# gevaertlab/sequoia-pub

Measured on AMD Instinct MI355X. Metric: slides/sec (1000-patch WSI, UNI-dim, 20k-gene head), higher is better.
Workload: dtype f16x3; 1 GPU; pipeline: 1000 x 224x224 uint8 patches/slide -> ResNet-50 embed -> k-Means(100) -> ViS(D=2048, depth 6, 16 heads, G=20820) forward (BASELINE config 3), patches uploaded from pinned host memory every step; embedder=ResNet-50 (src/resnet.py forward_extract), feature_dim=2048, patch_size=224, parallelism=slide-sharded x1

## Files before the change

### sequoia-pub_amd/csrc/gemm.h

```cpp
#pragma once
#include "sq_common.h"

#define SQ_ACT_NONE 0
#define SQ_ACT_GELU 1
#define SQ_ACT_RELU 2

struct GemmArgs {
    const void* A = nullptr;
    const void* B = nullptr;
    void* C = nullptr;
    bf16_t* C2 = nullptr;
    void* Cpre = nullptr;
    const float* bias = nullptr;
    const float* rowbias = nullptr;
    const void* res = nullptr;
    const void* gelu_grad_of = nullptr;
    const float* ln64_g = nullptr;
    const float* ln64_b = nullptr;
    float alpha = 1.0f;
    float* colsum_a = nullptr;
    int M = 0, N = 0, K = 0;
    int lda = 0, ldb = 0, ldc = 0, ldc2 = 0, ldpre = 0, ldres = 0, ldrb = 0, ldgg = 0;
    int rows_per_group = 1;
    int act = SQ_ACT_NONE;
    int out_dtype = SQ_F32, res_dtype = SQ_F32, pre_dtype = SQ_F32, gg_dtype = SQ_F32;
    int batch = 1;
    long long sA = 0, sB = 0, sC = 0, sC2 = 0, sPre = 0, sBias = 0, sRb = 0, sRes = 0, sGg = 0;
    int conv = 0, H = 0, W = 0, Cin = 0, OH = 0, OW = 0, KW = 1, stride = 1, pad = 0;
    size_t a_bytes = 0, b_bytes = 0;
    long long plA = 0, plB = 0, plRes = 0, plC = 0;
    int x3_f16 = 0;
    const float* colscale = nullptr;
    float* splitk_ws = nullptr;
    size_t splitk_ws_bytes = 0;
    int splitk = 1;
    int ngroup = 0;
    const void* gA[4] = {nullptr, nullptr, nullptr, nullptr};
    const void* gB[4] = {nullptr, nullptr, nullptr, nullptr};
    void* gC[4] = {nullptr, nullptr, nullptr, nullptr};
    float* gcs[4] = {nullptr, nullptr, nullptr, nullptr};
    int vec_epi = 0;
    int b_tiled = 0;
    const void* A2 = nullptr; long long plA2 = 0; size_t a2_bytes = 0; int lda2 = 0;
    const void* B2 = nullptr; size_t b2_bytes = 0; int ldb2 = 0; int K2 = 0;
    const float* bias2 = nullptr; const float* colscale2 = nullptr;
    int dH = 0, dW = 0, dOH = 0, dOW = 0, dstride = 1;
    int tile_group_m = 0;
    const void* comb_w = nullptr;
    const float* comb_rb = nullptr;
    int comb_ldrb = 0, comb_rpg = 1;
    int dbg = 0;
};

template <typename P>
static __device__ __forceinline__ P sq_group_pick(P const (&a)[4], int i) { return i == 0 ? a[0] : i == 1 ? a[1] : i == 2 ? a[2] : a[3]; }

int sq_launch_gemm(const GemmArgs& a, int dtype, hipStream_t stream);
bool sq_gemm_takes_p8_256(const GemmArgs& a);
int sq_launch_gemm_x3(const GemmArgs& a, hipStream_t stream);
int sq_launch_gemm_tn(const GemmArgs& a, int dtype, hipStream_t stream);
int sq_launch_splitk_reduce(const GemmArgs& a, hipStream_t stream);
```

### sequoia-pub_amd/csrc/gemm_x3.hip

```cpp
#include "gemm.h"
#include "x3_fmt.h"
#include "cdna_prims.h"

#include <cstdio>
#include <cstdlib>

extern int g_x3_small_max_k;
bool sq_conv_halo_x3_eligible(const GemmArgs& a);
int sq_launch_conv_halo_x3(const GemmArgs& a, hipStream_t stream);
extern int g_x3_halo;
extern int g_dbg;

namespace {

__device__ __forceinline__ u32x4 ld16(const bf16_t* p) { return *reinterpret_cast<const u32x4*>(p); }
__device__ __forceinline__ void st16(bf16_t* p, const u32x4& v) { *reinterpret_cast<u32x4*>(p) = v; }

constexpr int BK = 32, ROWB = 64;
constexpr int WTM = 2;

template <int BM_, int WTN> struct X3Cfg {
    static constexpr int BM = BM_;
    static constexpr int NT = BM_ * 2;
    static constexpr int BN = 64 * WTN;
    static constexpr int A_BYTES = BM * ROWB;
    static constexpr int B_BYTES = BN * ROWB;
    static constexpr int STAGE_BYTES = 2 * A_BYTES + 2 * B_BYTES;
    static constexpr int NSTAGE = BM_ == 256 ? 3 : 2;
    static constexpr int EPI_BYTES = BM * BN * 4;
    static constexpr int LDS_BYTES = NSTAGE * STAGE_BYTES > EPI_BYTES ? NSTAGE * STAGE_BYTES : EPI_BYTES;
    static constexpr int ROUND = NT / 4;
    static constexpr bool SPLIT_B = BN < ROUND;
    static constexpr int RB = SPLIT_B ? 1 : 2 * (BN / ROUND);
    static constexpr int LOADS = 4 + RB;
};

template <int BM_, int WTN, bool CONV, bool F16, bool PP, bool DUAL = false, bool UNI = false>
__global__ __launch_bounds__(BM_ * 2, BM_ == 256 ? 1 : 2) void gemm_x3_kernel(const GemmArgs p) {
    static_assert(!DUAL || (BM_ == 128 && !CONV && !PP), "the dual form lives in the 128-row two-stage shape");
    static_assert(!UNI || (F16 && !CONV && !DUAL), "the UNI epilogues are fp16-plane plain products");
    using Cfg = X3Cfg<BM_, WTN>;
    using Fmt = X3Fmt<F16>;
    constexpr int BM = Cfg::BM, NT = Cfg::NT, A_BYTES = Cfg::A_BYTES, ROUND = Cfg::ROUND;
    constexpr int BN = Cfg::BN, B_BYTES = Cfg::B_BYTES, STAGE_BYTES = Cfg::STAGE_BYTES, NSTAGE = Cfg::NSTAGE;
    static_assert(!PP || BM_ == 256, "the ping-pong schedule needs the 8-wave block");
    extern __shared__ __attribute__((aligned(16))) char smem[];

    const int tid = threadIdx.x, lane = tid & 63;
    const int wave = __builtin_amdgcn_readfirstlane(tid >> 6);
    const int wm = wave >> 1, wn = wave & 1;

    const int tiles_n = (p.N + BN - 1) / BN, tiles_m = (p.M + BM - 1) / BM;
    const int nwg = tiles_m * tiles_n;
    const int t = sq_xcd_tile(blockIdx.x, nwg);
    const int m0 = (t / tiles_n) * BM, n0 = (t % tiles_n) * BN;

    const bf16_t* Ah = reinterpret_cast<const bf16_t*>(p.A);
    const bf16_t* Bh = reinterpret_cast<const bf16_t*>(p.B);
    const auto rsAh = sq_rsrc(Ah, (int)p.a_bytes);
    const auto rsAl = sq_rsrc(Ah + p.plA, (int)p.a_bytes);
    const auto rsBh = sq_rsrc(Bh, (int)p.b_bytes);
    const auto rsBl = sq_rsrc(Bh + p.plB, (int)p.b_bytes);

    const int r0 = tid >> 2;
    const int gc = (tid & 3) ^ ((r0 >> 2) & 3);
    uint32_t a_off[2];
    int a_ih0[2], a_iw0[2];
    uint32_t a_pix[2];
    bool a_ok[2];
#pragma unroll
    for (int j = 0; j < 2; ++j) {
        const int m = m0 + r0 + ROUND * j;
        a_ok[j] = m < p.M;
        if constexpr (CONV) {
            const int ohw = p.OH * p.OW;
            const int img = m / ohw;
            const int rem = m - img * ohw;
            const int oh = rem / p.OW, ow = rem - oh * p.OW;
            a_ih0[j] = oh * p.stride - p.pad;
            a_iw0[j] = ow * p.stride - p.pad;
            a_pix[j] = (uint32_t)(img * p.H * p.W);
            a_off[j] = 0;
        } else {
            a_ih0[j] = a_iw0[j] = 0;
            a_pix[j] = 0;
            a_off[j] = a_ok[j] ? ((uint32_t)m * (uint32_t)p.lda + (uint32_t)(gc * 8)) * 2u : SQ_OOB;
        }
    }
    constexpr int RBP = Cfg::SPLIT_B ? 1 : BN / ROUND;
    uint32_t b_off[RBP];
    const bool b_lo_half = Cfg::SPLIT_B && r0 >= 64;
#pragma unroll
    for (int j = 0; j < RBP; ++j) {
        const int n = n0 + (Cfg::SPLIT_B ? (r0 & 63) : r0 + ROUND * j);
        b_off[j] = n >= p.N ? SQ_OOB : p.b_tiled ? ((uint32_t)n * 32u + (uint32_t)(gc * 8)) * 2u : ((uint32_t)n * (uint32_t)p.ldb + (uint32_t)(gc * 8)) * 2u;
    }
    auto issue_loads = [&](int kt, int buf) {
        const int k0 = kt * BK;
        const bool k_ok = k0 + gc * 8 < p.K;
        char* sa = smem + buf * STAGE_BYTES + wave * 1024;
        char* sb = sa + 2 * A_BYTES;
        if constexpr (CONV) {
            const int tap = k0 / p.Cin;
            const int cin0 = k0 - tap * p.Cin + gc * 8;
            const int kh = tap / p.KW, kw = tap - kh * p.KW;
#pragma unroll
// ... 282 lines not shown
            }
#pragma unroll
            for (int j = 0; j < WTN; ++j) {
                const int col = min(n0 + wn * (WTN * 32) + j * 32 + l31, p.N - 1);
                const float s3 = p.colscale ? p.alpha * p.colscale[col] : p.alpha, b3 = p.bias ? p.bias[col] : 0.f;
                const float sd = p.colscale2 ? p.colscale2[col] : 1.f, bd = p.bias2 ? p.bias2[col] : 0.f;
#pragma unroll
                for (int i = 0; i < WTM; ++i)
#pragma unroll
                    for (int r = 0; r < 16; r += 2) {
                        const float d0 = sd * accd[i][j][r] + bd, d1 = sd * accd[i][j][r + 1] + bd;
                        const uint32_t h = Fmt::pack2(d0, d1);
                        const uint32_t l = Fmt::rest2(d0, d1, h);
                        acc[i][j][r] = x3_relu((s3 * acc[i][j][r] + b3) + Fmt::sum_lo(h, l));
                        acc[i][j][r + 1] = x3_relu((s3 * acc[i][j][r + 1] + b3) + Fmt::sum_hi(h, l));
                    }
            }
        }
    }
    __syncthreads();

    float* stage = reinterpret_cast<float*>(smem);
#pragma unroll
    for (int i = 0; i < WTM; ++i)
#pragma unroll
        for (int j = 0; j < WTN; ++j)
#pragma unroll
            for (int r = 0; r < 16; ++r) {
                const int row = wm * (WTM * 32) + i * 32 + (r & 3) + 8 * (r >> 2) + 4 * lh;
                const int col = wn * (WTN * 32) + j * 32 + l31;
                stage[row * BN + col] = acc[i][j][r];
            }
    __syncthreads();
    if (!e_live) return;

    const bf16_t* resh = (!UNI && p.res) ? reinterpret_cast<const bf16_t*>(p.res) : nullptr;
    const float* res32 = (UNI && p.res) ? reinterpret_cast<const float*>(p.res) : nullptr;
    bf16_t* ch = p.out_dtype != SQ_F32 ? reinterpret_cast<bf16_t*>(p.C) : nullptr;
    float* c32 = p.out_dtype == SQ_F32 ? reinterpret_cast<float*>(p.C) : nullptr;
    constexpr int U = 4;
    u32x4 nh[U], nl[U];
    const bool res_nxt = res_pre && ITER == 2 * U && NPRE == U;
    if (res_nxt) {
#pragma unroll
        for (int u = 0; u < U; ++u) {
            const int m = min(m0 + e_rbase + (U + u) * RPI, p.M - 1);
            nh[u] = ld16(resh + (long long)m * p.ldres + e_n);
            nl[u] = ld16(resh + p.plRes + (long long)m * p.ldres + e_n);
        }
    }
#pragma unroll
    for (int c0 = 0; c0 < ITER; c0 += U) {
        u32x4 rh[U], rl[U];
#pragma unroll
        for (int u = 0; u < U; ++u) {
            rh[u] = u32x4{0, 0, 0, 0}; rl[u] = u32x4{0, 0, 0, 0};
            const int m = m0 + e_rbase + (c0 + u) * RPI;
            if constexpr (BM_ == 128) {
                if (res_pre && c0 + u < NPRE) { rh[u] = rpre_h[c0 + u]; rl[u] = rpre_l[c0 + u]; continue; }
                if (res_nxt && c0 == U) { rh[u] = nh[u]; rl[u] = nl[u]; continue; }
            }
            if (resh && m < p.M) {
                rh[u] = ld16(resh + (long long)m * p.ldres + e_n);
                rl[u] = ld16(resh + p.plRes + (long long)m * p.ldres + e_n);
            }
        }
#pragma unroll
        for (int u = 0; u < U; ++u) {
            const int row = e_rbase + (c0 + u) * RPI;
            const int m = m0 + row;
            if (m >= p.M) continue;
            const f32x4 a0 = *reinterpret_cast<const f32x4*>(stage + row * BN + e_c8 * 8);
            const f32x4 a1 = *reinterpret_cast<const f32x4*>(stage + row * BN + e_c8 * 8 + 4);
            float v[8] = {a0[0], a0[1], a0[2], a0[3], a1[0], a1[1], a1[2], a1[3]};
            if constexpr (!DUAL) {
#pragma unroll
            for (int e = 0; e < 8; ++e) v[e] = scale8[e] * v[e] + bias8[e];
            if (resh) {
                float idn[8];
                x3_join8<F16>(rh[u], rl[u], idn);
#pragma unroll
                for (int e = 0; e < 8; ++e) v[e] += idn[e];
            }
            if constexpr (UNI) {
                if (res32) {
                    const float* r = res32 + (long long)m * p.ldres + e_n;
                    const f32x4 r0 = *reinterpret_cast<const f32x4*>(r), r1 = *reinterpret_cast<const f32x4*>(r + 4);
#pragma unroll
                    for (int e = 0; e < 4; ++e) { v[e] += r0[e]; v[4 + e] += r1[e]; }
                }
                if (p.act == SQ_ACT_GELU) {
#pragma unroll
                    for (int e = 0; e < 8; ++e) v[e] = sq_gelu<false>(v[e]);
                }
            }
            if (p.act == SQ_ACT_RELU) {
#pragma unroll
                for (int e = 0; e < 8; ++e) v[e] = x3_relu(v[e]);
            }
            }
            if (p.dbg & 1) continue;
            if (c32) {
                float* d = c32 + (long long)m * p.ldc + e_n;
                *reinterpret_cast<f32x4*>(d) = f32x4{v[0], v[1], v[2], v[3]};
                *reinterpret_cast<f32x4*>(d + 4) = f32x4{v[4], v[5], v[6], v[7]};
            }
            if (ch) {
                u32x4 hi, lo;
                x3_split8<F16>(v, hi, lo);
                st16(ch + (long long)m * p.ldc + e_n, hi);
                st16(ch + p.plC + (long long)m * p.ldc + e_n, lo);
            }
        }
    }
}

template <int BM_, int WTN, bool F16, bool PP>
int launch_x3(const GemmArgs& a, hipStream_t stream) {
    using Cfg = X3Cfg<BM_, WTN>;
    static SqDevOnce attr;
    if (attr.needed()) {
        SQ_HIP_CHECK(hipFuncSetAttribute((const void*)gemm_x3_kernel<BM_, WTN, false, F16, PP>, hipFuncAttributeMaxDynamicSharedMemorySize, Cfg::LDS_BYTES));
        SQ_HIP_CHECK(hipFuncSetAttribute((const void*)gemm_x3_kernel<BM_, WTN, true, F16, PP>, hipFuncAttributeMaxDynamicSharedMemorySize, Cfg::LDS_BYTES));
        attr.done();
    }
    const int tiles = ((a.M + BM_ - 1) / BM_) * ((a.N + Cfg::BN - 1) / Cfg::BN);
    const dim3 grid(tiles), block(Cfg::NT);
    if (a.conv) hipLaunchKernelGGL((gemm_x3_kernel<BM_, WTN, true, F16, PP>), grid, block, Cfg::LDS_BYTES, stream, a);
    else hipLaunchKernelGGL((gemm_x3_kernel<BM_, WTN, false, F16, PP>), grid, block, Cfg::LDS_BYTES, stream, a);
    SQ_LAUNCH_CHECK();
    return SQ_OK;
}

template <bool F16>
int launch_x3_dual(const GemmArgs& a, hipStream_t stream) {
    using Cfg = X3Cfg<128, 2>;
    static SqDevOnce attr;
    if (attr.needed()) {
        SQ_HIP_CHECK(hipFuncSetAttribute((const void*)gemm_x3_kernel<128, 2, false, F16, false, true>, hipFuncAttributeMaxDynamicSharedMemorySize, Cfg::LDS_BYTES));
        attr.done();
    }
    const int tiles = ((a.M + 127) / 128) * (a.N / Cfg::BN);
    hipLaunchKernelGGL((gemm_x3_kernel<128, 2, false, F16, false, true>), dim3(tiles), dim3(Cfg::NT), Cfg::LDS_BYTES, stream, a);
    SQ_LAUNCH_CHECK();
    return SQ_OK;
}

template <int BM_, int WTN, bool PP>
int launch_x3_uni(const GemmArgs& a, hipStream_t stream) {
    using Cfg = X3Cfg<BM_, WTN>;
    static SqDevOnce attr;
    if (attr.needed()) {
        SQ_HIP_CHECK(hipFuncSetAttribute((const void*)gemm_x3_kernel<BM_, WTN, false, true, PP, false, true>, hipFuncAttributeMaxDynamicSharedMemorySize, Cfg::LDS_BYTES));
        attr.done();
    }
    const int tiles = ((a.M + BM_ - 1) / BM_) * ((a.N + Cfg::BN - 1) / Cfg::BN);
    hipLaunchKernelGGL((gemm_x3_kernel<BM_, WTN, false, true, PP, false, true>), dim3(tiles), dim3(Cfg::NT), Cfg::LDS_BYTES, stream, a);
    SQ_LAUNCH_CHECK();
    return SQ_OK;
}

template <int BM_, bool PP>
int launch_x3_uni_fmt(const GemmArgs& a, hipStream_t stream) {
    return a.N % 128 == 0 ? launch_x3_uni<BM_, 2, PP>(a, stream) : launch_x3_uni<BM_, 1, PP>(a, stream);
}

template <int BM_, bool PP>
int launch_x3_fmt(const GemmArgs& a, hipStream_t stream) {
    if (a.x3_f16) return a.N % 128 == 0 ? launch_x3<BM_, 2, true, PP>(a, stream) : launch_x3<BM_, 1, true, PP>(a, stream);
    return a.N % 128 == 0 ? launch_x3<BM_, 2, false, PP>(a, stream) : launch_x3<BM_, 1, false, PP>(a, stream);
}

}

int sq_launch_gemm_x3(const GemmArgs& a_in, hipStream_t stream) {
    GemmArgs a = a_in;
    a.dbg |= g_dbg;
    SQ_REQUIRE(a.M > 0 && a.N > 0 && a.K > 0 && a.batch == 1, "gemm_x3: empty or batched problem M=%d N=%d K=%d batch=%d", a.M, a.N, a.K, a.batch);
    SQ_REQUIRE(a.K % 8 == 0 && a.ldb % 8 == 0 && a.N % 8 == 0, "gemm_x3: K=%d / ldb=%d / N=%d must be multiples of 8", a.K, a.ldb, a.N);
    SQ_REQUIRE(a.plA != 0 && a.plB != 0 && (a.plA & 7) == 0 && (a.plB & 7) == 0, "gemm_x3: operand plane strides must be non-zero multiples of 8 elements");
    SQ_REQUIRE(((uintptr_t)a.A & 15) == 0 && ((uintptr_t)a.B & 15) == 0 && ((uintptr_t)a.C & 15) == 0, "gemm_x3: A/B/C must be 16-byte aligned");
    SQ_REQUIRE(a.a_bytes > 0 && a.a_bytes < (1ull << 31) && a.b_bytes > 0 && a.b_bytes < (1ull << 31),
               "gemm_x3: operand plane extents must be in (0, 2 GiB): %zu %zu", a.a_bytes, a.b_bytes);
    SQ_REQUIRE(a.out_dtype == SQ_F32 || ((a.out_dtype == SQ_BF16X3 || a.out_dtype == SQ_F16X3) && a.plC != 0 && (a.plC & 7) == 0), "gemm_x3: output is fp32 or hi/lo planes (plC)");
    const bool uni = a.act == SQ_ACT_GELU || (a.res && a.res_dtype == SQ_F32);
    SQ_REQUIRE(a.ldc % 8 == 0 && (!a.res || (a.res_dtype == SQ_F32 ? a.ldres % 4 == 0 && ((uintptr_t)a.res & 15) == 0
                                                                     : ((a.res_dtype == SQ_BF16X3 || a.res_dtype == SQ_F16X3) && a.ldres % 8 == 0 && a.plRes != 0 && (a.plRes & 7) == 0 && ((uintptr_t)a.res & 15) == 0))),
               "gemm_x3: ldc / residual must allow 16-byte accesses");
    SQ_REQUIRE(!a.rowbias && !a.Cpre && !a.gelu_grad_of && !a.ln64_g && !a.C2 && (a.act == SQ_ACT_NONE || a.act == SQ_ACT_RELU || a.act == SQ_ACT_GELU),
               "gemm_x3: only bias / residual / ReLU / GELU epilogues");
    SQ_REQUIRE(!uni || (a.x3_f16 && !a.conv && !a.A2 && a.act != SQ_ACT_RELU),
               "gemm_x3: the fp32-residual / GELU epilogues are for fp16-plane plain products without ReLU");
    SQ_REQUIRE((!a.bias || ((uintptr_t)a.bias & 15) == 0) && (!a.colscale || ((uintptr_t)a.colscale & 15) == 0), "gemm_x3: bias / colscale must be 16-byte aligned");
    SQ_REQUIRE(!a.b_tiled || a.K % BK == 0, "gemm_x3: K-tile-major weights need K %% %d == 0 (K=%d)", BK, a.K);
    if (a.conv) SQ_REQUIRE(a.Cin % BK == 0, "conv_x3: Cin=%d must be a multiple of the K-tile (%d)", a.Cin, BK);
    else SQ_REQUIRE(a.lda % 8 == 0, "gemm_x3: lda=%d must be a multiple of 8", a.lda);
    const bool dual = a.A2 != nullptr;
    if (dual) {
        SQ_REQUIRE(!a.conv && !a.res && a.act == SQ_ACT_RELU && a.N % 128 == 0 && a.out_dtype != SQ_F32, "gemm_x3 dual: plain product, no residual, ReLU, N %% 128 == 0, plane output");
        SQ_REQUIRE(a.B2 && a.K2 > 0 && a.K2 % BK == 0 && a.lda2 % 8 == 0 && a.plA2 != 0 && (a.plA2 & 7) == 0 && ((uintptr_t)a.A2 & 15) == 0 && ((uintptr_t)a.B2 & 15) == 0,
                   "gemm_x3 dual: second operand pair (K2=%d)", a.K2);
        SQ_REQUIRE(a.a2_bytes > 0 && a.a2_bytes < (1ull << 31) && a.b2_bytes > 0 && a.b2_bytes < (1ull << 31) && (a.b_tiled || a.ldb2 % 8 == 0), "gemm_x3 dual: operand extents");
        SQ_REQUIRE(a.dOH > 0 && a.dOW > 0 && a.M % (a.dOH * a.dOW) == 0 && a.dstride >= 1 && (a.dOH - 1) * a.dstride < a.dH && (a.dOW - 1) * a.dstride < a.dW,
                   "gemm_x3 dual: gather geometry %dx%d -> %dx%d stride %d", a.dH, a.dW, a.dOH, a.dOW, a.dstride);
    }
    SqProf prof(stream);
    if (prof.on() && dual) {
        char name[96];
        snprintf(name, sizeof(name), "dual_%s_M%d_N%d_K%d_K%d", a.x3_f16 ? "f16x3" : "bf16x3", a.M, a.N, a.K, a.K2);
        prof.begin(name, 2.0 * a.M * (double)a.N * (a.K + a.K2), ((double)a.M * (a.K + a.K2) + (double)a.N * (a.K + a.K2)) * 4.0 + (double)a.M * a.N * 4.0);
    } else if (prof.on()) {
        const double flops = 2.0 * a.M * (double)a.N * a.K;
        const double a_elems = a.conv ? (double)a.M / (a.OH * a.OW) * a.H * a.W * a.Cin : (double)a.M * a.K;
        const double bytes = (a_elems + (double)a.N * a.K) * 4.0 + (double)a.M * a.N * (4.0 + (a.res ? 4.0 : 0.0));
        char name[96];
        snprintf(name, sizeof(name), "%s_%s_M%d_N%d_K%d", a.conv ? "conv" : "gemm", a.x3_f16 ? "f16x3" : "bf16x3", a.M, a.N, a.K);
        prof.begin(name, flops, bytes);
    }
    const int small_max_k = g_x3_small_max_k >= 0 ? g_x3_small_max_k : 256;
    const bool small = a.K <= small_max_k || (a.N <= 64 && small_max_k > 0);
    return uni ? (small ? launch_x3_uni_fmt<128, false>(a, stream) : launch_x3_uni_fmt<256, true>(a, stream))
         : dual ? (a.x3_f16 ? launch_x3_dual<true>(a, stream) : launch_x3_dual<false>(a, stream))
         : (g_x3_halo != 0 && sq_conv_halo_x3_eligible(a)) ? sq_launch_conv_halo_x3(a, stream)
         : (a.K <= small_max_k || (a.N <= 64 && small_max_k > 0)) ? launch_x3_fmt<128, false>(a, stream)
         : launch_x3_fmt<256, true>(a, stream);
}

extern "C" int sq_linear_x3(int fmt, const void* A_hi, const void* A_lo, int lda, const void* W_hi, const void* W_lo, int ldw, const float* bias,
                            const float* colscale, const void* res_hi, const void* res_lo, int ldres, int act, void* C_hi, void* C_lo, float* C_f32, int ldc,
                            int M, int N, int K, const int* conv_geom, void* stream) {
    SQ_REQUIRE(A_hi && A_lo && W_hi && W_lo && ((C_hi && C_lo) != (C_f32 != nullptr)), "linear_x3: null pointer (give C_hi + C_lo or C_f32)");
    SQ_REQUIRE((res_hi == nullptr) == (res_lo == nullptr), "linear_x3: residual needs both planes");
    SQ_REQUIRE(fmt == 0 || fmt == 1, "linear_x3: fmt %d (0 = bf16 planes, 1 = fp16 planes)", fmt);
    GemmArgs g;
    g.x3_f16 = fmt; g.colscale = colscale;
    const int xdt = fmt ? SQ_F16X3 : SQ_BF16X3;
    g.M = M; g.N = N; g.K = K;
    g.A = A_hi; g.plA = (const bf16_t*)A_lo - (const bf16_t*)A_hi; g.lda = lda;
    g.B = W_hi; g.plB = (const bf16_t*)W_lo - (const bf16_t*)W_hi; g.ldb = ldw;
    g.b_bytes = ((size_t)(N - 1) * ldw + K) * 2;
    if (conv_geom) {
        g.conv = 1; g.H = conv_geom[1]; g.W = conv_geom[2]; g.Cin = conv_geom[3]; g.OH = conv_geom[4]; g.OW = conv_geom[5];
        g.KW = conv_geom[6]; g.stride = conv_geom[7]; g.pad = conv_geom[8];
        SQ_REQUIRE(M == conv_geom[0] * g.OH * g.OW && g.Cin > 0 && K % g.Cin == 0, "linear_x3: inconsistent convolution geometry");
        g.a_bytes = (size_t)conv_geom[0] * g.H * g.W * g.Cin * 2;
    } else {
        g.a_bytes = ((size_t)(M - 1) * lda + K) * 2;
    }
    g.bias = bias; g.act = act;
    if (res_hi) { g.res = res_hi; g.plRes = (const bf16_t*)res_lo - (const bf16_t*)res_hi; g.ldres = ldres; g.res_dtype = xdt; }
    if (C_f32) { g.C = C_f32; g.out_dtype = SQ_F32; }
    else { g.C = C_hi; g.plC = (bf16_t*)C_lo - (bf16_t*)C_hi; g.out_dtype = xdt; }
    g.ldc = ldc;
    return sq_launch_gemm_x3(g, (hipStream_t)stream);
}
```

### sequoia-pub_amd/csrc/resnet.hip

```cpp
#include "../../include/sequoia_hip.h"
#include "gemm.h"
#include "x3_fmt.h"

int sq_launch_bottleneck_tail_c64(const bf16_t* t1, const bf16_t* res, bf16_t* y, bf16_t* t1n, int cn,
                                  const bf16_t* w2, const bf16_t* w3, const bf16_t* w1n, size_t w2_bytes, size_t w3_bytes, size_t w1n_bytes,
                                  const float* b2, const float* b3, const float* b1n,
                                  const bf16_t* xin, const bf16_t* wd, size_t wd_bytes, const float* bd,
                                  int n_img, int H, int W, hipStream_t stream);
int sq_launch_bottleneck_chain_c256(const bf16_t* t2, const bf16_t* res, bf16_t* y, bf16_t* t1n, const bf16_t* w3,
                                    const bf16_t* w1n, size_t w3_bytes, size_t w1n_bytes, const float* b3, const float* b1n,
                                    long long P, hipStream_t stream);
int sq_launch_bottleneck_chain_c128(const bf16_t* t2, const bf16_t* res, bf16_t* y, bf16_t* t1n, int cn, const bf16_t* w3,
                                    const bf16_t* w1n, size_t w3_bytes, size_t w1n_bytes, const float* b3, const float* b1n,
                                    long long P, hipStream_t stream);
int sq_launch_conv1_pool_bf16(const uint8_t* u8, const float* f32_nchw, const bf16_t* w152, const float* bias, bf16_t* out,
                              int n, int H, int W, hipStream_t stream);
int sq_launch_chain_x3_c64(int f16, const uint16_t* t2, long long plT2, const uint16_t* res, long long plRes, uint16_t* y, long long plY,
                           uint16_t* t1n, long long plT1n, int n2, const uint16_t* w3, const uint16_t* w1n, long long plW, size_t w3_bytes,
                           const float* b3, const float* cs3, const float* b1n, const float* cs1n,
                           const uint16_t* xin, long long plX, const uint16_t* wd, size_t wd_bytes, const float* bd, const float* csd,
                           const uint16_t* t1, long long plT1, const uint16_t* w2, size_t w2_bytes, const float* b2, const float* cs2, int W, int HW,
                           long long P, uint16_t* frag, int w_tiled, hipStream_t stream);
size_t sq_chain_x3_frag_bytes();
bool sq_chain_x3w_eligible(int c, int n2);
// ... 102 lines not shown
            for (int e = 0; e < 4; ++e) o[e] = (__float_as_uint(best[2 * e]) >> 16) | (__float_as_uint(best[2 * e + 1]) & 0xffff0000u);
        } else {
#pragma unroll
            for (int e = 0; e < 4; ++e) o[e] = __float_as_uint(best[e]);
        }
        *reinterpret_cast<u32x4*>(out + (size_t)px * C + cg * V) = o;
    }
}

template <typename T>
__global__ void avgpool7_kernel(const T* __restrict__ in, float* __restrict__ out, int n, int H, int W, int C) {
    const int idx = blockIdx.x * blockDim.x + threadIdx.x;
    if (idx >= n * C) return;
    const int c = idx % C, img = idx / C;
    float acc = 0.f;
    for (int h = 0; h < 7; ++h)
        for (int w = 0; w < 7; ++w) acc += ldf(in + (((size_t)img * H + h) * W + w) * C + c);
    out[idx] = acc / 49.0f;
}


template <bool F16>
__global__ void avgpool7_x3_kernel(const bf16_t* __restrict__ in, long long plane, float* __restrict__ out, int n, int H, int W, int C,
                                   unsigned* __restrict__ nonfinite) {
    const int idx = blockIdx.x * blockDim.x + threadIdx.x;
    if (idx >= n * C) return;
    const int c = idx % C, img = idx / C;
    float acc = 0.f;
    for (int h = 0; h < 7; ++h)
        for (int w = 0; w < 7; ++w) {
            const size_t o = (((size_t)img * H + h) * W + w) * C + c;
            acc += X3Fmt<F16>::one(in[o]) + X3Fmt<F16>::one(in[plane + o]);
        }
    out[idx] = acc / 49.0f;
    if (nonfinite && !(fabsf(acc) <= 3.0e38f)) atomicOr(nonfinite, 1u);
}

template <int MODE>
__global__ __launch_bounds__(256) void tap_copy_kernel(const void* __restrict__ src, long long plane, float* __restrict__ dst, size_t groups) {
    for (size_t g = (size_t)blockIdx.x * blockDim.x + threadIdx.x; g < groups; g += (size_t)gridDim.x * blockDim.x) {
        float v[8];
        if constexpr (MODE == 0) {
            const f32x4 a = *reinterpret_cast<const f32x4*>((const float*)src + g * 8), c = *reinterpret_cast<const f32x4*>((const float*)src + g * 8 + 4);
#pragma unroll
            for (int e = 0; e < 4; ++e) { v[e] = a[e]; v[4 + e] = c[e]; }
        } else if constexpr (MODE == 1) {
            const u32x4 t = *reinterpret_cast<const u32x4*>((const bf16_t*)src + g * 8);
#pragma unroll
            for (int e = 0; e < 4; ++e) { v[2 * e] = __uint_as_float(t[e] << 16); v[2 * e + 1] = __uint_as_float(t[e] & 0xffff0000u); }
        } else {
            const uint16_t* h = (const uint16_t*)src + g * 8;
            const u32x4 hi = *reinterpret_cast<const u32x4*>(h), lo = *reinterpret_cast<const u32x4*>(h + plane);
            const uint16_t* hs = reinterpret_cast<const uint16_t*>(&hi);
            const uint16_t* ls = reinterpret_cast<const uint16_t*>(&lo);
#pragma unroll
            for (int e = 0; e < 8; ++e) v[e] = X3Fmt<MODE == 3>::one(hs[e]) + X3Fmt<MODE == 3>::one(ls[e]);
        }
        *reinterpret_cast<f32x4*>(dst + g * 8) = f32x4{v[0], v[1], v[2], v[3]};
        *reinterpret_cast<f32x4*>(dst + g * 8 + 4) = f32x4{v[4], v[5], v[6], v[7]};
    }
}

struct RnTaps { float* out; const int64_t* off; };

struct ConvSpec { int cin, cout, k, stride, pad; };

void build_specs(ConvSpec* specs) {
    int i = 0;
// ... 133 lines not shown
    SQ_REQUIRE(dtype == SQ_F32 || dtype == SQ_BF16 || dtype == SQ_BF16X3 || dtype == SQ_F16X3, "resnet50: dtype %d", dtype);
    SQ_REQUIRE(weights && bias && features && workspace, "resnet50: null pointer");
    SQ_REQUIRE((patches_u8 != nullptr) != (patches_f32_nchw != nullptr), "resnet50: give exactly one of patches_u8 / patches_f32_nchw");
    if (hw_rule) {
        SQ_REQUIRE(n >= 1 && rn_hw_admitted(H0, W0),
                   "resnet50_hw: n=%d, patch %d x %d; height and width must each lie in [%d, %d] -- the sizes whose final map is 7..13 per axis, "
                   "so that AvgPool2d(7) yields one window and 2048 features (above: the reference returns more; below: it fails)",
                   n, H0, W0, SQ_RESNET50_HW_MIN, SQ_RESNET50_HW_MAX);
    } else {
        SQ_REQUIRE(n >= 1 && H0 >= 224 && H0 % 32 == 0, "resnet50: n=%d patch_size=%d (need a multiple of 32, >= 224)", n, H0);
    }
    sq_resnet50_layout lay;
    sq_resnet50_layout_init(&lay);
    RnBufs b;
    rn_bufs(dtype, n, H0, W0, (char*)workspace, &b);
    if (b.bytes > workspace_bytes) {
        sq_set_error("resnet50: workspace %zu < required %zu", workspace_bytes, b.bytes);
        return SQ_ERR_WORKSPACE;
    }
    const bool x3 = dtype == SQ_BF16X3 || dtype == SQ_F16X3;
    const bool f16 = dtype == SQ_F16X3;
    const float* colscale = x3 ? bias + lay.b_total : nullptr;
    const size_t es = x3 ? 2 : sq_dtype_size(dtype);
    const bool lp = dtype == SQ_BF16;
    auto W = [&](const sq_conv_desc& d) { return (const void*)((const char*)weights + (size_t)d.w_off * es); };
    const size_t w_bytes_total = (size_t)lay.w_total * es;
    const int OH1 = (H0 + 1) / 2, OW1 = (W0 + 1) / 2;
    const size_t act_cap = (size_t)n * rn_act_elems(H0, W0) * es;
    const long long act_plane = (long long)n * (long long)rn_act_elems(H0, W0);
    SQ_REQUIRE(act_cap < (1ull << 31) && (lp || x3 || (size_t)n * OH1 * OW1 * CONV1_KP * es < (1ull << 31)),
               "resnet50: sub-batch of %d patches exceeds the 2 GiB buffer-descriptor limit (bf16 and the split modes: <= 1300 patches of 224, fp32: <= 280)", n);

    auto conv = [&](const sq_conv_desc& d, const void* in, int H, int Wd, void* out, int OH, int OW, const void* res, int act,
                    const sq_conv_desc* dd = nullptr, const void* din = nullptr, int dH = 0, int dW = 0) -> int {
        GemmArgs g;
        g.M = n * OH * OW; g.N = d.cout; g.K = d.k_padded;
        g.A = in;
        if (d.k == 1 && d.stride == 1) {
            g.lda = d.cin; g.a_bytes = (size_t)g.M * d.cin * es;
        } else {
            g.conv = 1; g.H = H; g.W = Wd; g.Cin = d.cin; g.OH = OH; g.OW = OW; g.KW = d.k; g.stride = d.stride; g.pad = d.pad;
            g.a_bytes = (size_t)n * H * Wd * d.cin * es;
        }
        g.B = W(d); g.ldb = d.k_padded; g.b_bytes = w_bytes_total - (size_t)d.w_off * es;
        g.bias = bias + d.b_off;
        g.res = res; g.ldres = d.cout; g.res_dtype = dtype;
        g.act = act;
        g.C = out; g.ldc = d.cout; g.out_dtype = dtype;
        if (x3) {
            g.plA = act_plane; g.plC = act_plane; g.plRes = act_plane; g.plB = lay.w_total;
            g.x3_f16 = f16; g.colscale = colscale + d.b_off;
            g.b_tiled = 1;
            if (dd) {
                g.A2 = din; g.plA2 = act_plane; g.lda2 = dd->cin; g.a2_bytes = (size_t)n * dH * dW * dd->cin * es;
                g.B2 = W(*dd); g.ldb2 = dd->k_padded; g.b2_bytes = w_bytes_total - (size_t)dd->w_off * es; g.K2 = dd->k_padded;
                g.bias2 = bias + dd->b_off; g.colscale2 = colscale + dd->b_off;
                g.dH = dH; g.dW = dW; g.dOH = OH; g.dOW = OW; g.dstride = dd->stride;
            }
            return sq_launch_gemm_x3(g, st);
        }
        return sq_launch_gemm(g, dtype, st);
    };
#define RUN(expr) do { if (int _e = (expr)) return _e; } while (0)
    auto tap = [&](int idx, const void* src) -> int {
        if (!taps) return SQ_OK;
        const size_t groups = (size_t)(taps->off[idx + 1] - taps->off[idx]) / 8;
        float* dst = taps->out + taps->off[idx];
        size_t nb = (groups + 255) / 256; if (nb > 65535) nb = 65535;
        if (f16) hipLaunchKernelGGL(tap_copy_kernel<3>, dim3((int)nb), dim3(256), 0, st, src, act_plane, dst, groups);
        else if (x3) hipLaunchKernelGGL(tap_copy_kernel<2>, dim3((int)nb), dim3(256), 0, st, src, act_plane, dst, groups);
        else if (lp) hipLaunchKernelGGL(tap_copy_kernel<1>, dim3((int)nb), dim3(256), 0, st, src, act_plane, dst, groups);
        else hipLaunchKernelGGL(tap_copy_kernel<0>, dim3((int)nb), dim3(256), 0, st, src, act_plane, dst, groups);
        SQ_LAUNCH_CHECK();
        return SQ_OK;
    };

    int H = (OH1 + 1) / 2, Wd = (OW1 + 1) / 2;
    bool stem_t1 = false;
    if (lp) {
        const sq_conv_desc& d = lay.conv[0];
        RUN(sq_launch_conv1_pool_bf16(patches_u8, patches_f32_nchw, (const bf16_t*)W(d), bias + d.b_off, (bf16_t*)b.act[1], n, H0, W0, st));
    } else if (x3) {
        const sq_conv_desc& d = lay.conv[0];
        const sq_conv_desc& r1 = lay.conv[1];
        stem_t1 = r1.k == 1 && r1.stride == 1 && r1.cin == 64 && r1.cout == 64 && !sq_env_flag("SQ_RESNET_NO_STEM_REDUCE");
        RUN(sq_launch_conv1_pool_x3(f16, patches_u8, patches_f32_nchw, (const uint16_t*)W(d), lay.w_total, bias + d.b_off, colscale + d.b_off,
                                    (uint16_t*)b.act[1], act_plane, n, H0, W0, st,
                                    stem_t1 ? (const uint16_t*)W(r1) : nullptr, 1, stem_t1 ? bias + r1.b_off : nullptr,
                                    stem_t1 ? colscale + r1.b_off : nullptr, stem_t1 ? (uint16_t*)b.act[2] : nullptr));
    } else {
        {
            const size_t work = (size_t)n * OH1 * OW1 * (CONV1_KP / 8);
            size_t nb = (work + 255) / 256; if (nb > 65535) nb = 65535;
            hipLaunchKernelGGL(im2col_conv1_kernel<float>, dim3((int)nb), dim3(256), 0, st, patches_u8, patches_f32_nchw, (float*)b.col, n, H0, W0, OH1, OW1);
            SQ_LAUNCH_CHECK();
            GemmArgs g;
            const sq_conv_desc& d = lay.conv[0];
            g.M = n * OH1 * OW1; g.N = 64; g.K = CONV1_KP;
            g.A = b.col; g.lda = CONV1_KP; g.a_bytes = (size_t)g.M * CONV1_KP * es;
            g.B = W(d); g.ldb = CONV1_KP; g.b_bytes = w_bytes_total;
            g.bias = bias + d.b_off; g.act = SQ_ACT_RELU;
            g.C = b.act[0]; g.ldc = 64; g.out_dtype = dtype;
            RUN(sq_launch_gemm(g, dtype, st));
        }
        {
            const size_t work = (size_t)n * H * Wd * 64 / (16 / es);
            size_t nb = (work + 255) / 256; if (nb > 65535) nb = 65535;
            hipLaunchKernelGGL(maxpool3x3s2_kernel<float>, dim3((int)nb), dim3(256), 0, st, (const float*)b.act[0], (float*)b.act[1], n, OH1, OW1, H, Wd, 64);
            SQ_LAUNCH_CHECK();
        }
    }
    const bool fuse56 = lp && !sq_env_flag("SQ_RESNET_NO_FUSE") && (128 + 2 * Wd + 2) * 128 <= 32768;
    const bool fuse_chain = lp && !sq_env_flag("SQ_RESNET_NO_FUSE") && !sq_env_flag("SQ_RESNET_NO_CHAIN");
    const bool fuse_chain256 = fuse_chain;
    int xi = 1, ci = 1, t1i = stem_t1 ? 2 : -1;
    const int blocks[4] = {3, 4, 6, 3};
    int blk = 0;
    for (int li = 0; li < 4; ++li)
        for (int bk = 0; bk < blocks[li]; ++bk, ++blk) {
            int free_[4], nf = 0;
            for (int i = 0; i < 5; ++i) if (i != xi && i != t1i) free_[nf++] = i;
            void* x = b.act[xi];
            const int t1_idx = t1i >= 0 ? t1i : free_[--nf];
            void* t1 = b.act[t1_idx];
            const sq_conv_desc& c1 = lay.conv[ci]; const sq_conv_desc& c2 = lay.conv[ci + 1]; const sq_conv_desc& c3 = lay.conv[ci + 2];
            const bool has_ds = bk == 0;
            const int OH = (H - 1) / c2.stride + 1, OW = (Wd - 1) / c2.stride + 1;
            RUN(tap(2 * blk, x));
            if (t1i < 0) RUN(conv(c1, x, H, Wd, t1, H, Wd, nullptr, SQ_ACT_RELU));
            RUN(tap(2 * blk + 1, t1));
            const int cnext = ci + (has_ds ? 4 : 3);
            if (fuse56 && li == 0) {
                void* y = b.act[free_[1]]; void* t1n = b.act[free_[2]];
                const sq_conv_desc& n1 = lay.conv[cnext];
                const sq_conv_desc& dsd = lay.conv[ci + 3];
                auto rest = [&](const sq_conv_desc& d) { return w_bytes_total - (size_t)d.w_off * es; };
                RUN(sq_launch_bottleneck_tail_c64((const bf16_t*)t1, has_ds ? nullptr : (const bf16_t*)x, (bf16_t*)y, (bf16_t*)t1n, n1.cout,
                                                  (const bf16_t*)W(c2), (const bf16_t*)W(c3), (const bf16_t*)W(n1), rest(c2), rest(c3), rest(n1),
                                                  bias + c2.b_off, bias + c3.b_off, bias + n1.b_off,
                                                  has_ds ? (const bf16_t*)x : nullptr, has_ds ? (const bf16_t*)W(dsd) : nullptr,
                                                  has_ds ? rest(dsd) : 0, has_ds ? bias + dsd.b_off : nullptr, n, H, Wd, st));
                xi = free_[1];
                t1i = free_[2];
                ci = cnext;
                continue;
            }
            void* t2 = b.act[free_[0]]; void* ds = b.act[free_[1]]; void* y = b.act[free_[2]];
            const bool x3_chain = x3 && !sq_env_flag("SQ_RESNET_NO_CHAIN") && c3.cin == 64 && c3.cout == 256 && c2.stride == 1 &&
                cnext < SQ_RESNET50_CONVS && lay.conv[cnext].k == 1 && lay.conv[cnext].stride == 1 && lay.conv[cnext].cin == 256 &&
                (lay.conv[cnext].cout == 64 || lay.conv[cnext].cout == 128) &&
// ... 36 lines not shown
            const void* identity = x;
            const bool x3_dual = x3 && has_ds && lay.conv[ci + 3].k == 1 && c3.k == 1 && c3.cout % 128 == 0 && !sq_env_flag("SQ_RESNET_NO_DUAL");
            if (has_ds && !x3_dual) {
                RUN(conv(lay.conv[ci + 3], x, H, Wd, ds, OH, OW, nullptr, SQ_ACT_NONE));
                identity = ds;
            }
            if (fuse_chain && c3.cin == 128 && c3.cout == 512 && cnext < SQ_RESNET50_CONVS && lay.conv[cnext].k == 1 &&
                lay.conv[cnext].cin == 512 && (lay.conv[cnext].cout == 128 || lay.conv[cnext].cout == 256)) {
                const sq_conv_desc& n1 = lay.conv[cnext];
                auto rest = [&](const sq_conv_desc& d) { return w_bytes_total - (size_t)d.w_off * es; };
                RUN(sq_launch_bottleneck_chain_c128((const bf16_t*)t2, (const bf16_t*)identity, (bf16_t*)y, (bf16_t*)t1, n1.cout,
                                                    (const bf16_t*)W(c3), (const bf16_t*)W(n1), rest(c3), rest(n1), bias + c3.b_off,
                                                    bias + n1.b_off, (long long)n * OH * OW, st));
                ci = cnext;
                xi = free_[2];
                t1i = t1_idx;
                H = OH; Wd = OW;
                continue;
            }
            if (fuse_chain256 && c3.cin == 256 && c3.cout == 1024 && cnext < SQ_RESNET50_CONVS && lay.conv[cnext].k == 1 &&
                lay.conv[cnext].cin == 1024 && lay.conv[cnext].cout == 256) {
                const sq_conv_desc& n1 = lay.conv[cnext];
                auto rest = [&](const sq_conv_desc& d) { return w_bytes_total - (size_t)d.w_off * es; };
                RUN(sq_launch_bottleneck_chain_c256((const bf16_t*)t2, (const bf16_t*)identity, (bf16_t*)y, (bf16_t*)t1,
                                                    (const bf16_t*)W(c3), (const bf16_t*)W(n1), rest(c3), rest(n1), bias + c3.b_off,
                                                    bias + n1.b_off, (long long)n * OH * OW, st));
                ci = cnext;
                xi = free_[2];
                t1i = t1_idx;
                H = OH; Wd = OW;
                continue;
            }
            if (x3_dual) RUN(conv(c3, t2, OH, OW, y, OH, OW, nullptr, SQ_ACT_RELU, &lay.conv[ci + 3], x, H, Wd));
            else RUN(conv(c3, t2, OH, OW, y, OH, OW, identity, SQ_ACT_RELU));
            ci = cnext;
            xi = free_[2];
            t1i = -1;
            H = OH; Wd = OW;
        }
    RUN(tap(2 * blk, b.act[xi]));
    {
        const int total = n * 2048;
        if (f16) hipLaunchKernelGGL(avgpool7_x3_kernel<true>, dim3((total + 255) / 256), dim3(256), 0, st, (const bf16_t*)b.act[xi], act_plane, features, n, H, Wd, 2048, nonfinite_flag);
        else if (x3) hipLaunchKernelGGL(avgpool7_x3_kernel<false>, dim3((total + 255) / 256), dim3(256), 0, st, (const bf16_t*)b.act[xi], act_plane, features, n, H, Wd, 2048, nonfinite_flag);
        else if (lp) hipLaunchKernelGGL(avgpool7_kernel<bf16_t>, dim3((total + 255) / 256), dim3(256), 0, st, (const bf16_t*)b.act[xi], features, n, H, Wd, 2048);
        else hipLaunchKernelGGL(avgpool7_kernel<float>, dim3((total + 255) / 256), dim3(256), 0, st, (const float*)b.act[xi], features, n, H, Wd, 2048);
        SQ_LAUNCH_CHECK();
    }
#undef RUN
    (void)act_cap;
    return SQ_OK;
}
```

### sequoia-pub_amd/csrc/x3_fmt.h

```cpp
#pragma once
#include "cdna_prims.h"

typedef _Float16 f16x8 __attribute__((ext_vector_type(8)));
typedef _Float16 f16x2 __attribute__((ext_vector_type(2)));

template <bool F16> struct X3Fmt;

template <> struct X3Fmt<false> {
    static __device__ __forceinline__ uint32_t pack2(float a, float b) { return pack_bf16x2(a, b); }
    static __device__ __forceinline__ float lo_f(uint32_t u) { return __uint_as_float(u << 16); }
    static __device__ __forceinline__ float hi_f(uint32_t u) { return __uint_as_float(u & 0xffff0000u); }
    static __device__ __forceinline__ float one(uint16_t h) { return __uint_as_float(((uint32_t)h) << 16); }
    static __device__ __forceinline__ float sum_lo(uint32_t h, uint32_t l) { return lo_f(h) + lo_f(l); }
    static __device__ __forceinline__ float sum_hi(uint32_t h, uint32_t l) { return hi_f(h) + hi_f(l); }
    static __device__ __forceinline__ uint32_t rest2(float a, float b, uint32_t h) { return pack2(a - lo_f(h), b - hi_f(h)); }
    static __device__ __forceinline__ void mma(const u32x4& a, const u32x4& b, f32x16& acc) { acc = mfma_bf16(a, b, acc); }
};

template <> struct X3Fmt<true> {
    static __device__ __forceinline__ uint32_t pack2(float a, float b) {
        const sq_f32x2 v = {a, b};
        return __builtin_bit_cast(uint32_t, __builtin_convertvector(v, f16x2));
    }
    static __device__ __forceinline__ float lo_f(uint32_t u) { return (float)__builtin_bit_cast(f16x2, u)[0]; }
    static __device__ __forceinline__ float hi_f(uint32_t u) { return (float)__builtin_bit_cast(f16x2, u)[1]; }
    static __device__ __forceinline__ float one(uint16_t h) { return (float)__builtin_bit_cast(_Float16, h); }
    static __device__ __forceinline__ float sum_lo(uint32_t h, uint32_t l) {
        float r; asm("v_fma_mix_f32 %0, %1, 1.0, %2 op_sel:[0,0,0] op_sel_hi:[1,0,1]" : "=v"(r) : "v"(h), "v"(l)); return r;
    }
    static __device__ __forceinline__ float sum_hi(uint32_t h, uint32_t l) {
        float r; asm("v_fma_mix_f32 %0, %1, 1.0, %2 op_sel:[1,0,1] op_sel_hi:[1,0,1]" : "=v"(r) : "v"(h), "v"(l)); return r;
    }
    static __device__ __forceinline__ uint32_t rest2(float a, float b, uint32_t h) {
        float ra, rb;
        asm("v_fma_mix_f32 %0, %1, -1.0, %2 op_sel:[0,0,0] op_sel_hi:[1,0,0]" : "=v"(ra) : "v"(h), "v"(a));
        asm("v_fma_mix_f32 %0, %1, -1.0, %2 op_sel:[1,0,0] op_sel_hi:[1,0,0]" : "=v"(rb) : "v"(h), "v"(b));
        return pack2(ra, rb);
    }
    static __device__ __forceinline__ void mma(const u32x4& a, const u32x4& b, f32x16& acc) {
        union { u32x4 u; f16x8 h; } ua, ub;
        ua.u = a; ub.u = b;
        acc = __builtin_amdgcn_mfma_f32_32x32x16_f16(ua.h, ub.h, acc, 0, 0, 0);
    }
};

__device__ __forceinline__ float x3_relu(float v) { return v < 0.f ? 0.f : v; }

template <bool F16>
__device__ __forceinline__ void x3_split8(const float (&v)[8], u32x4& hi, u32x4& lo) {
    using F = X3Fmt<F16>;
#pragma unroll
    for (int e = 0; e < 4; ++e) {
        hi[e] = F::pack2(v[2 * e], v[2 * e + 1]);
        lo[e] = F::rest2(v[2 * e], v[2 * e + 1], hi[e]);
    }
}
template <bool F16>
__device__ __forceinline__ void x3_join8(const u32x4& hi, const u32x4& lo, float (&v)[8]) {
    using F = X3Fmt<F16>;
#pragma unroll
    for (int e = 0; e < 4; ++e) {
        v[2 * e] = F::sum_lo(hi[e], lo[e]);
        v[2 * e + 1] = F::sum_hi(hi[e], lo[e]);
    }
}
```

Before: 34.41 slides/s.

## Fuse ResNet final 7x7 average pool into last bottleneck conv GEMM epilogue

Adds a pooled variant of the x3 GEMM kernel whose tiles are aligned to whole 7x7 feature maps (five images per 256-row tile). The epilogue applies residual and ReLU, rounds through the hi/lo split to match the stored activation, writes the values to LDS, then reduces each map to the pooled feature directly. This is used for the last ResNet block's conv3, so the final activation never has to be written to memory and read back by a separate avgpool kernel. In exchange, each tile leaves 11 of its 256 rows unused (245 live), and the final activation buffer is no longer produced.

```diff
diff --git a/sequoia-pub_amd/csrc/gemm.h b/sequoia-pub_amd/csrc/gemm.h
--- a/sequoia-pub_amd/csrc/gemm.h
+++ b/sequoia-pub_amd/csrc/gemm.h
@@ -50,6 +50,9 @@
     const float* comb_rb = nullptr;
     int comb_ldrb = 0, comb_rpg = 1;
     int dbg = 0;
+    float* pool_out = nullptr;
+    int pool_H = 0, pool_W = 0;
+    unsigned* pool_flag = nullptr;
 };
 
 template <typename P>
@@ -58,5 +61,6 @@
 int sq_launch_gemm(const GemmArgs& a, int dtype, hipStream_t stream);
 bool sq_gemm_takes_p8_256(const GemmArgs& a);
 int sq_launch_gemm_x3(const GemmArgs& a, hipStream_t stream);
+bool sq_gemm_x3_pool_eligible(const GemmArgs& a);
 int sq_launch_gemm_tn(const GemmArgs& a, int dtype, hipStream_t stream);
 int sq_launch_splitk_reduce(const GemmArgs& a, hipStream_t stream);
diff --git a/sequoia-pub_amd/csrc/gemm_x3.hip b/sequoia-pub_amd/csrc/gemm_x3.hip
--- a/sequoia-pub_amd/csrc/gemm_x3.hip
+++ b/sequoia-pub_amd/csrc/gemm_x3.hip
@@ -35,10 +35,11 @@
     static constexpr int LOADS = 4 + RB;
 };
 
-template <int BM_, int WTN, bool CONV, bool F16, bool PP, bool DUAL = false, bool UNI = false>
+template <int BM_, int WTN, bool CONV, bool F16, bool PP, bool DUAL = false, bool UNI = false, bool POOL = false>
 __global__ __launch_bounds__(BM_ * 2, BM_ == 256 ? 1 : 2) void gemm_x3_kernel(const GemmArgs p) {
     static_assert(!DUAL || (BM_ == 128 && !CONV && !PP), "the dual form lives in the 128-row two-stage shape");
     static_assert(!UNI || (F16 && !CONV && !DUAL), "the UNI epilogues are fp16-plane plain products");
+    static_assert(!POOL || (BM_ == 256 && !CONV && !DUAL && !UNI), "the pooled form is a plain product of the 256-row shape");
     using Cfg = X3Cfg<BM_, WTN>;
     using Fmt = X3Fmt<F16>;
     constexpr int BM = Cfg::BM, NT = Cfg::NT, A_BYTES = Cfg::A_BYTES, ROUND = Cfg::ROUND;
@@ -50,10 +51,12 @@
     const int wave = __builtin_amdgcn_readfirstlane(tid >> 6);
     const int wm = wave >> 1, wn = wave & 1;
 
-    const int tiles_n = (p.N + BN - 1) / BN, tiles_m = (p.M + BM - 1) / BM;
+    const int pool_r = POOL ? p.pool_H * p.pool_W : 1, pool_pt = POOL ? BM / pool_r : 1;
+    const int tile_rows = POOL ? pool_pt * pool_r : BM;
+    const int tiles_n = (p.N + BN - 1) / BN, tiles_m = POOL ? (p.M / pool_r + pool_pt - 1) / pool_pt : (p.M + BM - 1) / BM;
     const int nwg = tiles_m * tiles_n;
     const int t = sq_xcd_tile(blockIdx.x, nwg);
-    const int m0 = (t / tiles_n) * BM, n0 = (t % tiles_n) * BN;
+    const int m0 = (t / tiles_n) * tile_rows, n0 = (t % tiles_n) * BN;
 
     const bf16_t* Ah = reinterpret_cast<const bf16_t*>(p.A);
     const bf16_t* Bh = reinterpret_cast<const bf16_t*>(p.B);
@@ -71,7 +74,7 @@
 #pragma unroll
     for (int j = 0; j < 2; ++j) {
         const int m = m0 + r0 + ROUND * j;
-        a_ok[j] = m < p.M;
+        a_ok[j] = m < p.M && (!POOL || r0 + ROUND * j < tile_rows);
         if constexpr (CONV) {
             const int ohw = p.OH * p.OW;
             const int img = m / ohw;
@@ -420,7 +423,9 @@
                 stage[row * BN + col] = acc[i][j][r];
             }
     __syncthreads();
-    if (!e_live) return;
+    if constexpr (!POOL) {
+        if (!e_live) return;
+    }
 
     const bf16_t* resh = (!UNI && p.res) ? reinterpret_cast<const bf16_t*>(p.res) : nullptr;
     const float* res32 = (UNI && p.res) ? reinterpret_cast<const float*>(p.res) : nullptr;
@@ -448,7 +453,7 @@
                 if (res_pre && c0 + u < NPRE) { rh[u] = rpre_h[c0 + u]; rl[u] = rpre_l[c0 + u]; continue; }
                 if (res_nxt && c0 == U) { rh[u] = nh[u]; rl[u] = nl[u]; continue; }
             }
-            if (resh && m < p.M) {
+            if (resh && m < p.M && (!POOL || (e_live && e_rbase + (c0 + u) * RPI < tile_rows))) {
                 rh[u] = ld16(resh + (long long)m * p.ldres + e_n);
                 rl[u] = ld16(resh + p.plRes + (long long)m * p.ldres + e_n);
             }
@@ -458,6 +463,9 @@
             const int row = e_rbase + (c0 + u) * RPI;
             const int m = m0 + row;
             if (m >= p.M) continue;
+            if constexpr (POOL) {
+                if (!e_live || row >= tile_rows) continue;
+            }
             const f32x4 a0 = *reinterpret_cast<const f32x4*>(stage + row * BN + e_c8 * 8);
             const f32x4 a1 = *reinterpret_cast<const f32x4*>(stage + row * BN + e_c8 * 8 + 4);
             float v[8] = {a0[0], a0[1], a0[2], a0[3], a1[0], a1[1], a1[2], a1[3]};
@@ -486,6 +494,18 @@
 #pragma unroll
                 for (int e = 0; e < 8; ++e) v[e] = x3_relu(v[e]);
             }
+            }
+            if constexpr (POOL) {
+                u32x4 hi, lo;
+                x3_split8<F16>(v, hi, lo);
+#pragma unroll
+                for (int e = 0; e < 4; ++e) {
+                    v[2 * e] = Fmt::one((uint16_t)(hi[e] & 0xffffu)) + Fmt::one((uint16_t)(lo[e] & 0xffffu));
+                    v[2 * e + 1] = Fmt::one((uint16_t)(hi[e] >> 16)) + Fmt::one((uint16_t)(lo[e] >> 16));
+                }
+                *reinterpret_cast<f32x4*>(stage + row * BN + e_c8 * 8) = f32x4{v[0], v[1], v[2], v[3]};
+                *reinterpret_cast<f32x4*>(stage + row * BN + e_c8 * 8 + 4) = f32x4{v[4], v[5], v[6], v[7]};
+                continue;
             }
             if (p.dbg & 1) continue;
             if (c32) {
@@ -499,6 +519,19 @@
                 st16(ch + (long long)m * p.ldc + e_n, hi);
                 st16(ch + p.plC + (long long)m * p.ldc + e_n, lo);
             }
+        }
+    }
+    if constexpr (POOL) {
+        __syncthreads();
+        const int n_img = p.M / pool_r, img0 = (t / tiles_n) * pool_pt;
+        for (int o = tid; o < pool_pt * BN; o += NT) {
+            const int pt = o / BN, c = o - pt * BN;
+            if (img0 + pt >= n_img || n0 + c >= p.N) continue;
+            const float* s = stage + pt * pool_r * BN + c;
+            float sum = 0.f;
+            for (int h = 0; h < 7; ++h)
+                for (int w = 0; w < 7; ++w) sum += s[(h * p.pool_W + w) * BN];
+            p.pool_out[(long long)(img0 + pt) * p.N + n0 + c] = x3_pool7_finish(sum, p.pool_flag);
         }
     }
 }
@@ -534,6 +567,27 @@
     return SQ_OK;
 }
 
+template <bool F16>
+int launch_x3_pool(const GemmArgs& a, hipStream_t stream) {
+    using Cfg = X3Cfg<256, 2>;
+    static SqDevOnce attr;
+    if (attr.needed()) {
+        SQ_HIP_CHECK(hipFuncSetAttribute((const void*)gemm_x3_kernel<256, 2, false, F16, true, false, false, true>, hipFuncAttributeMaxDynamicSharedMemorySize, Cfg::LDS_BYTES));
+        attr.done();
+    }
+    const int r = a.pool_H * a.pool_W, pt = 256 / r, n_img = a.M / r;
+    const int tiles = ((n_img + pt - 1) / pt) * (a.N / Cfg::BN);
+    hipLaunchKernelGGL((gemm_x3_kernel<256, 2, false, F16, true, false, false, true>), dim3(tiles), dim3(Cfg::NT), Cfg::LDS_BYTES, stream, a);
+    SQ_LAUNCH_CHECK();
+    return SQ_OK;
+}
+
+bool x3_takes_small(const GemmArgs& a) {
+    const int small_max_k = g_x3_small_max_k >= 0 ? g_x3_small_max_k : 256;
+    return a.K <= small_max_k || (a.N <= 64 && small_max_k > 0);
+}
+bool x3_is_uni(const GemmArgs& a) { return a.act == SQ_ACT_GELU || (a.res && a.res_dtype == SQ_F32); }
+
 template <int BM_, int WTN, bool PP>
 int launch_x3_uni(const GemmArgs& a, hipStream_t stream) {
     using Cfg = X3Cfg<BM_, WTN>;
@@ -559,6 +613,11 @@
     return a.N % 128 == 0 ? launch_x3<BM_, 2, false, PP>(a, stream) : launch_x3<BM_, 1, false, PP>(a, stream);
 }
 
+}
+
+bool sq_gemm_x3_pool_eligible(const GemmArgs& a) {
+    return a.pool_out != nullptr && !a.conv && !a.A2 && !x3_is_uni(a) && !x3_takes_small(a) && a.N % 128 == 0 && a.pool_H >= 7 && a.pool_W >= 7 &&
+           a.pool_H * a.pool_W <= 256 && a.M > 0 && a.M % (a.pool_H * a.pool_W) == 0;
 }
 
 int sq_launch_gemm_x3(const GemmArgs& a_in, hipStream_t stream) {
@@ -571,7 +630,7 @@
     SQ_REQUIRE(a.a_bytes > 0 && a.a_bytes < (1ull << 31) && a.b_bytes > 0 && a.b_bytes < (1ull << 31),
                "gemm_x3: operand plane extents must be in (0, 2 GiB): %zu %zu", a.a_bytes, a.b_bytes);
     SQ_REQUIRE(a.out_dtype == SQ_F32 || ((a.out_dtype == SQ_BF16X3 || a.out_dtype == SQ_F16X3) && a.plC != 0 && (a.plC & 7) == 0), "gemm_x3: output is fp32 or hi/lo planes (plC)");
-    const bool uni = a.act == SQ_ACT_GELU || (a.res && a.res_dtype == SQ_F32);
+    const bool uni = x3_is_uni(a);
     SQ_REQUIRE(a.ldc % 8 == 0 && (!a.res || (a.res_dtype == SQ_F32 ? a.ldres % 4 == 0 && ((uintptr_t)a.res & 15) == 0
                                                                      : ((a.res_dtype == SQ_BF16X3 || a.res_dtype == SQ_F16X3) && a.ldres % 8 == 0 && a.plRes != 0 && (a.plRes & 7) == 0 && ((uintptr_t)a.res & 15) == 0))),
                "gemm_x3: ldc / residual must allow 16-byte accesses");
@@ -592,8 +651,16 @@
         SQ_REQUIRE(a.dOH > 0 && a.dOW > 0 && a.M % (a.dOH * a.dOW) == 0 && a.dstride >= 1 && (a.dOH - 1) * a.dstride < a.dH && (a.dOW - 1) * a.dstride < a.dW,
                    "gemm_x3 dual: gather geometry %dx%d -> %dx%d stride %d", a.dH, a.dW, a.dOH, a.dOW, a.dstride);
     }
+    const bool pool = a.pool_out != nullptr;
+    if (pool) SQ_REQUIRE(sq_gemm_x3_pool_eligible(a), "gemm_x3 pooled: needs a plain product of the 256-row shape (K=%d), N %% 128 == 0 and whole %d x %d maps of at most 256 rows (M=%d)",
+                         a.K, a.pool_H, a.pool_W, a.M);
     SqProf prof(stream);
-    if (prof.on() && dual) {
+    if (prof.on() && pool) {
+        char name[96];
+        snprintf(name, sizeof(name), "gemmpool_%s_M%d_N%d_K%d", a.x3_f16 ? "f16x3" : "bf16x3", a.M, a.N, a.K);
+        prof.begin(name, 2.0 * a.M * (double)a.N * a.K,
+                   ((double)a.M * a.K + (double)a.N * a.K) * 4.0 + (a.res ? (double)a.M * a.N * 4.0 : 0.0) + (double)(a.M / (a.pool_H * a.pool_W)) * a.N * 4.0);
+    } else if (prof.on() && dual) {
         char name[96];
         snprintf(name, sizeof(name), "dual_%s_M%d_N%d_K%d_K%d", a.x3_f16 ? "f16x3" : "bf16x3", a.M, a.N, a.K, a.K2);
         prof.begin(name, 2.0 * a.M * (double)a.N * (a.K + a.K2), ((double)a.M * (a.K + a.K2) + (double)a.N * (a.K + a.K2)) * 4.0 + (double)a.M * a.N * 4.0);
@@ -605,12 +672,12 @@
         snprintf(name, sizeof(name), "%s_%s_M%d_N%d_K%d", a.conv ? "conv" : "gemm", a.x3_f16 ? "f16x3" : "bf16x3", a.M, a.N, a.K);
         prof.begin(name, flops, bytes);
     }
-    const int small_max_k = g_x3_small_max_k >= 0 ? g_x3_small_max_k : 256;
-    const bool small = a.K <= small_max_k || (a.N <= 64 && small_max_k > 0);
-    return uni ? (small ? launch_x3_uni_fmt<128, false>(a, stream) : launch_x3_uni_fmt<256, true>(a, stream))
+    const bool small = x3_takes_small(a);
+    return pool ? (a.x3_f16 ? launch_x3_pool<true>(a, stream) : launch_x3_pool<false>(a, stream))
+         : uni ? (small ? launch_x3_uni_fmt<128, false>(a, stream) : launch_x3_uni_fmt<256, true>(a, stream))
          : dual ? (a.x3_f16 ? launch_x3_dual<true>(a, stream) : launch_x3_dual<false>(a, stream))
          : (g_x3_halo != 0 && sq_conv_halo_x3_eligible(a)) ? sq_launch_conv_halo_x3(a, stream)
-         : (a.K <= small_max_k || (a.N <= 64 && small_max_k > 0)) ? launch_x3_fmt<128, false>(a, stream)
+         : small ? launch_x3_fmt<128, false>(a, stream)
          : launch_x3_fmt<256, true>(a, stream);
 }
 
diff --git a/sequoia-pub_amd/csrc/resnet.hip b/sequoia-pub_amd/csrc/resnet.hip
--- a/sequoia-pub_amd/csrc/resnet.hip
+++ b/sequoia-pub_amd/csrc/resnet.hip
@@ -158,8 +158,7 @@
             const size_t o = (((size_t)img * H + h) * W + w) * C + c;
             acc += X3Fmt<F16>::one(in[o]) + X3Fmt<F16>::one(in[plane + o]);
         }
-    out[idx] = acc / 49.0f;
-    if (nonfinite && !(fabsf(acc) <= 3.0e38f)) atomicOr(nonfinite, 1u);
+    out[idx] = x3_pool7_finish(acc, nonfinite);
 }
 
 template <int MODE>
@@ -359,7 +358,7 @@
                "resnet50: sub-batch of %d patches exceeds the 2 GiB buffer-descriptor limit (bf16 and the split modes: <= 1300 patches of 224, fp32: <= 280)", n);
 
     auto conv = [&](const sq_conv_desc& d, const void* in, int H, int Wd, void* out, int OH, int OW, const void* res, int act,
-                    const sq_conv_desc* dd = nullptr, const void* din = nullptr, int dH = 0, int dW = 0) -> int {
+                    const sq_conv_desc* dd = nullptr, const void* din = nullptr, int dH = 0, int dW = 0, bool* pooled = nullptr) -> int {
         GemmArgs g;
         g.M = n * OH * OW; g.N = d.cout; g.K = d.k_padded;
         g.A = in;
@@ -383,6 +382,11 @@
                 g.B2 = W(*dd); g.ldb2 = dd->k_padded; g.b2_bytes = w_bytes_total - (size_t)dd->w_off * es; g.K2 = dd->k_padded;
                 g.bias2 = bias + dd->b_off; g.colscale2 = colscale + dd->b_off;
                 g.dH = dH; g.dW = dW; g.dOH = OH; g.dOW = OW; g.dstride = dd->stride;
+            }
+            if (pooled) {
+                g.pool_out = features; g.pool_H = OH; g.pool_W = OW; g.pool_flag = nonfinite_flag;
+                *pooled = sq_gemm_x3_pool_eligible(g);
+                if (!*pooled) g.pool_out = nullptr;
             }
             return sq_launch_gemm_x3(g, st);
         }
@@ -443,6 +447,8 @@
     int xi = 1, ci = 1, t1i = stem_t1 ? 2 : -1;
     const int blocks[4] = {3, 4, 6, 3};
     int blk = 0;
+    const bool pool_epi = x3 && !taps && !sq_env_flag("SQ_RESNET_NO_POOL_EPI");
+    bool pooled = false;
     for (int li = 0; li < 4; ++li)
         for (int bk = 0; bk < blocks[li]; ++bk, ++blk) {
             int free_[4], nf = 0;
@@ -545,6 +551,7 @@
                 continue;
             }
             if (x3_dual) RUN(conv(c3, t2, OH, OW, y, OH, OW, nullptr, SQ_ACT_RELU, &lay.conv[ci + 3], x, H, Wd));
+            else if (pool_epi && blk == 15) RUN(conv(c3, t2, OH, OW, y, OH, OW, identity, SQ_ACT_RELU, nullptr, nullptr, 0, 0, &pooled));
             else RUN(conv(c3, t2, OH, OW, y, OH, OW, identity, SQ_ACT_RELU));
             ci = cnext;
             xi = free_[2];
@@ -552,7 +559,7 @@
             H = OH; Wd = OW;
         }
     RUN(tap(2 * blk, b.act[xi]));
-    {
+    if (!pooled) {
         const int total = n * 2048;
         if (f16) hipLaunchKernelGGL(avgpool7_x3_kernel<true>, dim3((total + 255) / 256), dim3(256), 0, st, (const bf16_t*)b.act[xi], act_plane, features, n, H, Wd, 2048, nonfinite_flag);
         else if (x3) hipLaunchKernelGGL(avgpool7_x3_kernel<false>, dim3((total + 255) / 256), dim3(256), 0, st, (const bf16_t*)b.act[xi], act_plane, features, n, H, Wd, 2048, nonfinite_flag);
diff --git a/sequoia-pub_amd/csrc/x3_fmt.h b/sequoia-pub_amd/csrc/x3_fmt.h
--- a/sequoia-pub_amd/csrc/x3_fmt.h
+++ b/sequoia-pub_amd/csrc/x3_fmt.h
@@ -46,6 +46,11 @@
 
 __device__ __forceinline__ float x3_relu(float v) { return v < 0.f ? 0.f : v; }
 
+__device__ __forceinline__ float x3_pool7_finish(float acc, unsigned* nonfinite) {
+    if (nonfinite && !(fabsf(acc) <= 3.0e38f)) atomicOr(nonfinite, 1u);
+    return acc / 49.0f;
+}
+
 template <bool F16>
 __device__ __forceinline__ void x3_split8(const float (&v)[8], u32x4& hi, u32x4& lo) {
     using F = X3Fmt<F16>;
```

Measured after the change: 34.63 slides/s, median of 6. About the same (+0.6%).
